# andrewmilson/ministark

Measured on NVIDIA H100. Metric: ntt_field_ops_per_s, higher is better.
Workload: dtype u64

## Files before the change

### ministark_b200/csrc/dft.cuh

```cuda
#pragma once
#include "field.cuh"

namespace msntt {
using namespace gl;

template <bool INV>
__host__ __device__ __forceinline__ constexpr u64 w16(int k) {
    constexpr u64 F[8] = {0x00000000FFFFFFFFULL, 0x0000000010000000ULL, 0xFEFFFFFF01000001ULL, 0xFFEFFFFF00000001ULL,
                          0xFFFFFFFEFFFF0001ULL, 0x00000FFFFFFFF000ULL, 0x0000010000000000ULL, 0x0000000000000010ULL};
    constexpr u64 I[8] = {0x00000000FFFFFFFFULL, 0xFFFFFFFEFFFFFFF1ULL, 0xFFFFFEFF00000001ULL, 0xFFFFEFFF00001001ULL,
                          0x0000000000010000ULL, 0x0010000000000000ULL, 0x00FFFFFFFF000000ULL, 0xFFFFFFFEF0000001ULL};
    return INV ? I[k] : F[k];
}

struct W16Shift {
    int m;
    bool neg;
};
template <bool INV>
__host__ __device__ constexpr W16Shift w16_shift(int k) {
    constexpr W16Shift F[8] = {{0, false}, {28, false}, {88, true}, {52, true}, {16, true}, {76, false}, {40, false}, {4, false}};
    constexpr W16Shift I[8] = {{0, false}, {4, true}, {40, true}, {76, true}, {16, false}, {52, false}, {88, false}, {28, true}};
    return INV ? I[k] : F[k];
}
__host__ __device__ constexpr u64 pow2_mod_p(int m) {
    return m < 64 ? (1ULL << m) : ((1ULL << (m - 32)) - (1ULL << (m - 64)));
}
template <bool INV, int K>
__host__ __device__ constexpr bool w16_shift_ok() {
    constexpr W16Shift s = w16_shift<INV>(K);
    constexpr u64 v = pow2_mod_p(s.m);
    return (s.neg ? P - v : v) == w16<INV>(K);
}
static_assert(w16_shift_ok<false, 1>() && w16_shift_ok<false, 2>() && w16_shift_ok<false, 3>() && w16_shift_ok<false, 4>() &&
              w16_shift_ok<false, 5>() && w16_shift_ok<false, 6>() && w16_shift_ok<false, 7>(), "forward 16th roots");
static_assert(w16_shift_ok<true, 1>() && w16_shift_ok<true, 2>() && w16_shift_ok<true, 3>() && w16_shift_ok<true, 4>() &&
              w16_shift_ok<true, 5>() && w16_shift_ok<true, 6>() && w16_shift_ok<true, 7>(), "inverse 16th roots");

template <int V>
struct IC {
    static constexpr int value = V;
    __host__ __device__ constexpr operator int() const { return V; }
};
template <int I, int N, typename F>
__device__ __forceinline__ void static_for(F &&f) {
    if constexpr (I < N) {
        f(IC<I>{});
        static_for<I + 1, N>(f);
    }
}
__host__ __device__ constexpr int brev_c(int k, int bits) {
    int r = 0;
    for (int b = 0; b < bits; b++) r |= ((k >> b) & 1) << (bits - 1 - b);
    return r;
}

template <int B, bool INV, int S, int A>
struct Bfly {
    static __device__ __forceinline__ void run(u64 (&x)[1 << B]) {
        constexpr int span = 1 << (B - S);
        if constexpr ((A & span) == 0) {
            constexpr int j = brev_c(A >> (B - S + 1), S - 1);
            const u64 u = x[A], v = x[A + span];
            if constexpr (j == 0) {
                if constexpr (S == 1) {
                    x[A] = add_lc(u, v);
                    x[A + span] = sub_lc(u, v);
                } else {
                    x[A] = add_ll(u, v);
                    x[A + span] = sub_ll(u, v);
                }
            } else {
#ifdef MS_DFT_CONST_MUL
                constexpr u64 w = w16<INV>(j * (16 >> S));
                const u64 t = mul(v, w);
                x[A] = add_lc(u, t);
                x[A + span] = sub_lc(u, t);
#else
                constexpr W16Shift sh = w16_shift<INV>(j * (16 >> S));
                const u64 t = mul_pow2<sh.m>(v);
                if constexpr (sh.neg) {
                    x[A] = sub_lc(u, t);
                    x[A + span] = add_lc(u, t);
                } else {
                    x[A] = add_lc(u, t);
                    x[A + span] = sub_lc(u, t);
                }
#endif
            }
        }
        if constexpr (A + 1 < (1 << B))
            Bfly<B, INV, S, A + 1>::run(x);
        else if constexpr (S < B)
            Bfly<B, INV, S + 1, 0>::run(x);
    }
};
template <int B, bool INV>
__device__ __forceinline__ void dft_regs(u64 (&x)[1 << B]) {
    Bfly<B, INV, 1, 0>::run(x);
}

}
```

### ministark_b200/csrc/field.cuh

```cuda
#pragma once
#ifndef __CUDACC_RTC__
#include <cstdint>
#endif

namespace gl {

typedef unsigned long long u64;
typedef unsigned int u32;

constexpr u64 P = 0xFFFFFFFF00000001ULL;
constexpr u64 EPS = 0xFFFFFFFFULL;
constexpr u64 ONE = EPS;
constexpr u64 R2 = 0xFFFFFFFE00000001ULL;
constexpr u64 TWO = 0x1FFFFFFFEULL;

#if defined(__CUDACC__)
#define GL_DEV __device__ __forceinline__
#define GL_HD __host__ __device__ __forceinline__
#else
#define GL_DEV inline
#define GL_HD inline
#endif

#if defined(__CUDACC__) && (defined(MS_CANON_MAD) || defined(MS_ADD_MAD))
static __constant__ u32 kEpsOperand = 0xFFFFFFFFu;
#endif
#if defined(__CUDA_ARCH__) && defined(MS_CANON_MAD)
__device__ __forceinline__ u64 canon(u64 x) {
    u64 r;
    asm("{\n\t.reg .u32 x0, x1, t0, t1, c;\n\tmov.b64 {x0, x1}, %1;\n\tadd.cc.u32 t0, x0, 0xffffffff;\n\taddc.cc.u32 t1, x1, 0;\n\t"
        "addc.u32 c, 0, 0;\n\tmad.wide.u32 %0, c, %2, %1;\n\t}"
        : "=l"(r) : "l"(x), "r"(kEpsOperand));
    return r;
}
#else
GL_HD u64 canon(u64 x) {
    u32 x0 = (u32)x, x1 = (u32)(x >> 32);
    const bool c = (x1 == 0xFFFFFFFFu) && (x0 != 0);
    x0 -= c ? 1u : 0u;
    x1 = c ? 0u : x1;
    return ((u64)x1 << 32) | x0;
}
#endif

GL_HD u64 add(u64 a, u64 b) {
    u64 s = a + b;
    u64 t = s + EPS;
    return (s < a || t < s) ? t : s;
}
GL_HD u64 sub(u64 a, u64 b) {
    u64 d = a - b;
    return a < b ? d - EPS : d;
}
GL_HD u64 neg(u64 a) { return a ? P - a : 0; }

#if defined(__CUDA_ARCH__)
__device__ __forceinline__ u64 pack64(u32 lo, u32 hi) { u64 r; asm("mov.b64 %0, {%1,%2};" : "=l"(r) : "r"(lo), "r"(hi)); return r; }
__device__ __forceinline__ void unpack64(u64 v, u32 &lo, u32 &hi) { asm("mov.b64 {%0,%1}, %2;" : "=r"(lo), "=r"(hi) : "l"(v)); }
#if defined(MS_ADD_MAD)
__device__ __forceinline__ u64 add_lc(u64 a, u64 t) {
    u32 a0, a1, t0, t1;
    u64 r;
    unpack64(a, a0, a1); unpack64(t, t0, t1);
    asm("{\n\t.reg .u32 s0, s1, c;\n\t.reg .u64 s;\n\tadd.cc.u32 s0, %1, %3;\n\taddc.cc.u32 s1, %2, %4;\n\taddc.u32 c, 0, 0;\n\t"
        "mov.b64 s, {s0, s1};\n\tmad.wide.u32 %0, c, %5, s;\n\t}"
        : "=l"(r) : "r"(a0), "r"(a1), "r"(t0), "r"(t1), "r"(kEpsOperand));
    return r;
}
#else
__device__ __forceinline__ u64 add_lc(u64 a, u64 t) {
    u32 a0, a1, t0, t1, s0, s1;
    unpack64(a, a0, a1); unpack64(t, t0, t1);
    asm("{\n\t.reg .u32 c;\n\tadd.cc.u32 %0, %2, %4;\n\taddc.cc.u32 %1, %3, %5;\n\taddc.u32 c, 0, 0;\n\t"
        "sub.cc.u32 %0, %0, c;\n\tsubc.u32 %1, %1, 0;\n\tadd.u32 %1, %1, c;\n\t}"
        : "=r"(s0), "=r"(s1) : "r"(a0), "r"(a1), "r"(t0), "r"(t1));
    return pack64(s0, s1);
}
#endif
__device__ __forceinline__ u64 sub_lc(u64 a, u64 t) {
    u32 a0, a1, t0, t1, s0, s1;
    unpack64(a, a0, a1); unpack64(t, t0, t1);
    asm("{\n\t.reg .u32 m;\n\tsub.cc.u32 %0, %2, %4;\n\tsubc.cc.u32 %1, %3, %5;\n\tsubc.u32 m, 0, 0;\n\t"
        "sub.cc.u32 %0, %0, m;\n\tsubc.u32 %1, %1, 0;\n\t}"
        : "=r"(s0), "=r"(s1) : "r"(a0), "r"(a1), "r"(t0), "r"(t1));
    return pack64(s0, s1);
}
__device__ __forceinline__ u64 add_ll(u64 a, u64 t) {
    u32 a0, a1, t0, t1, s0, s1;
    unpack64(a, a0, a1); unpack64(t, t0, t1);
    asm("{\n\t.reg .u32 c, m;\n\tadd.cc.u32 %0, %2, %4;\n\taddc.cc.u32 %1, %3, %5;\n\taddc.u32 c, 0, 0;\n\tsub.u32 m, 0, c;\n\t"
        "add.cc.u32 %0, %0, m;\n\taddc.cc.u32 %1, %1, 0;\n\taddc.u32 c, 0, 0;\n\tsub.u32 m, 0, c;\n\t"
        "add.cc.u32 %0, %0, m;\n\taddc.u32 %1, %1, 0;\n\t}"
        : "=r"(s0), "=r"(s1) : "r"(a0), "r"(a1), "r"(t0), "r"(t1));
    return pack64(s0, s1);
}
__device__ __forceinline__ u64 sub_ll(u64 a, u64 t) {
    u32 a0, a1, t0, t1, s0, s1;
    unpack64(a, a0, a1); unpack64(t, t0, t1);
    asm("{\n\t.reg .u32 m;\n\tsub.cc.u32 %0, %2, %4;\n\tsubc.cc.u32 %1, %3, %5;\n\tsubc.u32 m, 0, 0;\n\t"
        "sub.cc.u32 %0, %0, m;\n\tsubc.cc.u32 %1, %1, 0;\n\tsubc.u32 m, 0, 0;\n\t"
        "sub.cc.u32 %0, %0, m;\n\tsubc.u32 %1, %1, 0;\n\t}"
        : "=r"(s0), "=r"(s1) : "r"(a0), "r"(a1), "r"(t0), "r"(t1));
    return pack64(s0, s1);
}
#else
inline u64 add_lc(u64 a, u64 t) {
    u64 s = a + t;
    return s < a ? s + EPS : s;
}
inline u64 sub_lc(u64 a, u64 t) {
    u64 d = a - t;
    return a < t ? d - EPS : d;
}
inline u64 add_ll(u64 a, u64 b) {
    u64 s = a + b;
    if (s < a) { u64 s2 = s + EPS; s = s2 < s ? s2 + EPS : s2; }
    return s;
}
inline u64 sub_ll(u64 a, u64 b) {
    u64 d = a - b;
    if (a < b) { u64 d2 = d - EPS; d = d < EPS ? d2 - EPS : d2; }
    return d;
}
#endif

GL_HD u64 mont_reduce(u64 hi, u64 lo) {
#if defined(__CUDA_ARCH__)
    u32 r0, r1, r2, r3, q0, q1;
    unpack64(lo, r0, r1); unpack64(hi, r2, r3);
    asm("{\n\t.reg .u32 A1, e, B0, B1, m;\n\t"
        "add.cc.u32 A1, %3, %2;\n\taddc.u32 e, 0, 0;\n\tadd.u32 e, e, A1;\n\t"
        "sub.cc.u32 B0, %2, e;\n\tsubc.u32 B1, A1, 0;\n\t"
        "sub.cc.u32 %0, %4, B0;\n\tsubc.cc.u32 %1, %5, B1;\n\tsubc.u32 m, 0, 0;\n\t"
        "sub.cc.u32 %0, %0, m;\n\tsubc.u32 %1, %1, 0;\n\t}"
        : "=&r"(q0), "=&r"(q1) : "r"(r0), "r"(r1), "r"(r2), "r"(r3));
    return pack64(q0, q1);
#else
    u64 a = lo + (lo << 32);
    u64 e = a < lo;
    u64 b = a - (a >> 32) - e;
    u64 r = hi - b;
    return hi < b ? r - EPS : r;
#endif
}
GL_HD u64 mul(u64 a, u64 b) {
#if defined(__CUDA_ARCH__)
    return mont_reduce(__umul64hi(a, b), a * b);
#else
    unsigned __int128 x = (unsigned __int128)a * b;
    return mont_reduce((u64)(x >> 64), (u64)x);
#endif
}
template <int M>
GL_HD u64 mul_pow2(u64 x) {
    static_assert(M > 0 && M < 96, "shift out of range");
    if constexpr (M < 64) {
        return mont_reduce(x >> (64 - M), x << M);
    } else {
        constexpr int k = M - 64;
        const u64 lo = x << k, hi = x >> (64 - k);
        return canon(add_lc(lo, (hi << 32) - hi));
    }
}
GL_HD u64 sqr(u64 a) { return mul(a, a); }
GL_HD u64 to_mont(u64 x_canon) { return mul(x_canon, R2); }
GL_HD u64 from_mont(u64 w) { return mul(w, 1); }

GL_HD u64 pow(u64 a, u64 e) {
    u64 r = ONE;
    while (e) {
        if (e & 1) r = mul(r, a);
        a = sqr(a);
        e >>= 1;
    }
    return r;
}
GL_HD u64 inv(u64 a) {
    u64 x1 = a;
    u64 x2 = mul(sqr(x1), x1);
    u64 x3 = mul(sqr(x2), x1);
    u64 x6 = x3; for (int i = 0; i < 3; i++) x6 = sqr(x6); x6 = mul(x6, x3);
    u64 x12 = x6; for (int i = 0; i < 6; i++) x12 = sqr(x12); x12 = mul(x12, x6);
    u64 x24 = x12; for (int i = 0; i < 12; i++) x24 = sqr(x24); x24 = mul(x24, x12);
    u64 x30 = x24; for (int i = 0; i < 6; i++) x30 = sqr(x30); x30 = mul(x30, x6);
    u64 x31 = mul(sqr(x30), x1);
    u64 x32 = mul(sqr(x31), x1);
    u64 r = x31;
    for (int i = 0; i < 33; i++) r = sqr(r);
    return mul(r, x32);
}

struct Fq3 {
    u64 c0, c1, c2;
};
GL_HD Fq3 fq3(u64 a) { return Fq3{a, 0, 0}; }
GL_HD Fq3 add(Fq3 a, Fq3 b) { return Fq3{add(a.c0, b.c0), add(a.c1, b.c1), add(a.c2, b.c2)}; }
GL_HD Fq3 sub(Fq3 a, Fq3 b) { return Fq3{sub(a.c0, b.c0), sub(a.c1, b.c1), sub(a.c2, b.c2)}; }
GL_HD Fq3 neg(Fq3 a) { return Fq3{neg(a.c0), neg(a.c1), neg(a.c2)}; }
GL_HD Fq3 mul(Fq3 a, u64 b) { return Fq3{mul(a.c0, b), mul(a.c1, b), mul(a.c2, b)}; }
GL_HD Fq3 mul(Fq3 a, Fq3 b) {
    u64 v0 = mul(a.c0, b.c0), v1 = mul(a.c1, b.c1), v2 = mul(a.c2, b.c2);
    u64 x12 = sub(sub(mul(add(a.c1, a.c2), add(b.c1, b.c2)), v1), v2);
    u64 x01 = sub(sub(mul(add(a.c0, a.c1), add(b.c0, b.c1)), v0), v1);
    u64 x02 = sub(sub(mul(add(a.c0, a.c2), add(b.c0, b.c2)), v0), v2);
    return Fq3{add(v0, add(x12, x12)), add(x01, add(v2, v2)), add(x02, v1)};
}
GL_HD Fq3 sqr(Fq3 a) { return mul(a, a); }
GL_HD Fq3 pow(Fq3 a, u64 e) {
    Fq3 r = fq3(ONE);
    while (e) {
        if (e & 1) r = mul(r, a);
        a = sqr(a);
        e >>= 1;
    }
    return r;
}
GL_HD Fq3 inv(Fq3 a) {
    u64 s0 = sub(sqr(a.c0), mul(TWO, mul(a.c1, a.c2)));
    u64 s1 = sub(mul(TWO, sqr(a.c2)), mul(a.c0, a.c1));
    u64 s2 = sub(sqr(a.c1), mul(a.c0, a.c2));
    u64 nrm = add(mul(a.c0, s0), mul(TWO, add(mul(a.c2, s1), mul(a.c1, s2))));
    u64 ni = inv(nrm);
    return Fq3{mul(s0, ni), mul(s1, ni), mul(s2, ni)};
}

}
```

Measured before the change: 852.8 billion.

## Use lazy 96-bit limb arithmetic in register DFT to skip per-butterfly reduction

Replaces the per-butterfly modular repair in the radix-16 register DFT with unreduced 96-bit three-limb accumulation. A 2^7·p bias is added to the first element so subtractions stay non-negative, and reduction happens once at the end. Power-of-two twiddle multiplies become limb shifts with folding. This cuts ALU work per butterfly but raises register pressure (3 words per element), which could cause spills or lower occupancy.

```diff
diff --git a/ministark_b200/csrc/dft.cuh b/ministark_b200/csrc/dft.cuh
--- a/ministark_b200/csrc/dft.cuh
+++ b/ministark_b200/csrc/dft.cuh
@@ -95,9 +95,48 @@
             Bfly<B, INV, S + 1, 0>::run(x);
     }
 };
+#ifndef MS_DFT_REPAIR_EACH
+constexpr u64 kBiasLo = P << 7;
+constexpr u32 kBiasHi = (u32)(P >> 57);
+static_assert(kBiasHi == 127 && kBiasLo == 0xFFFFFF8000000080ULL, "2^7 p");
+template <int B, bool INV, int S, int A>
+struct BflyL {
+    static __host__ __device__ __forceinline__ void run(L96 (&x)[1 << B]) {
+        constexpr int span = 1 << (B - S);
+        if constexpr ((A & span) == 0) {
+            constexpr int j = brev_c(A >> (B - S + 1), S - 1);
+            const L96 u = x[A], v = x[A + span];
+            if constexpr (j == 0) {
+                x[A] = l96_add(u, v);
+                x[A + span] = l96_sub(u, v);
+            } else {
+                constexpr W16Shift sh = w16_shift<INV>(j * (16 >> S));
+                constexpr int K = sh.m >= 64 ? sh.m - 64 : sh.m + 32;
+                constexpr bool neg = sh.neg != (sh.m < 64);
+                const L96 t = l96_mul_pow2<K>(v);
+                x[A] = neg ? l96_sub(u, t) : l96_add(u, t);
+                x[A + span] = neg ? l96_add(u, t) : l96_sub(u, t);
+            }
+        }
+        if constexpr (A + 1 < (1 << B))
+            BflyL<B, INV, S, A + 1>::run(x);
+        else if constexpr (S < B)
+            BflyL<B, INV, S + 1, 0>::run(x);
+    }
+};
+#endif
+
 template <int B, bool INV>
-__device__ __forceinline__ void dft_regs(u64 (&x)[1 << B]) {
+__host__ __device__ __forceinline__ void dft_regs(u64 (&x)[1 << B]) {
+#ifdef MS_DFT_REPAIR_EACH
     Bfly<B, INV, 1, 0>::run(x);
+#else
+    L96 y[1 << B];
+    for (int i = 0; i < (1 << B); i++) y[i] = l96(x[i]);
+    y[0] = l96_add(y[0], L96{(u32)kBiasLo, (u32)(kBiasLo >> 32), kBiasHi});
+    BflyL<B, INV, 1, 0>::run(y);
+    for (int i = 0; i < (1 << B); i++) x[i] = l96_reduce(y[i]);
+#endif
 }
 
 }
diff --git a/ministark_b200/csrc/field.cuh b/ministark_b200/csrc/field.cuh
--- a/ministark_b200/csrc/field.cuh
+++ b/ministark_b200/csrc/field.cuh
@@ -123,6 +123,60 @@
     return d;
 }
 #endif
+
+struct L96 {
+    u32 w0, w1, w2;
+};
+GL_HD L96 l96(u64 x) { return L96{(u32)x, (u32)(x >> 32), 0u}; }
+#if defined(__CUDA_ARCH__)
+__device__ __forceinline__ L96 l96_add(L96 a, L96 b) {
+    L96 r;
+    asm("add.cc.u32 %0, %3, %6;\n\taddc.cc.u32 %1, %4, %7;\n\taddc.u32 %2, %5, %8;"
+        : "=r"(r.w0), "=r"(r.w1), "=r"(r.w2) : "r"(a.w0), "r"(a.w1), "r"(a.w2), "r"(b.w0), "r"(b.w1), "r"(b.w2));
+    return r;
+}
+__device__ __forceinline__ L96 l96_sub(L96 a, L96 b) {
+    L96 r;
+    asm("sub.cc.u32 %0, %3, %6;\n\tsubc.cc.u32 %1, %4, %7;\n\tsubc.u32 %2, %5, %8;"
+        : "=r"(r.w0), "=r"(r.w1), "=r"(r.w2) : "r"(a.w0), "r"(a.w1), "r"(a.w2), "r"(b.w0), "r"(b.w1), "r"(b.w2));
+    return r;
+}
+#else
+inline L96 l96_add(L96 a, L96 b) {
+    const u64 s0 = (u64)a.w0 + b.w0, s1 = (u64)a.w1 + b.w1 + (s0 >> 32);
+    return L96{(u32)s0, (u32)s1, a.w2 + b.w2 + (u32)(s1 >> 32)};
+}
+inline L96 l96_sub(L96 a, L96 b) {
+    const u64 d0 = (u64)a.w0 - b.w0, d1 = (u64)a.w1 - b.w1 - (d0 >> 63);
+    return L96{(u32)d0, (u32)d1, a.w2 - b.w2 - (u32)(d1 >> 63)};
+}
+#endif
+template <int K>
+GL_HD L96 l96_mul_pow2(L96 v) {
+    static_assert(K > 0 && K < 96, "shift out of range");
+    constexpr int q = K / 32, r = K % 32;
+    u32 y0, y1, y2, y3;
+    if constexpr (r == 0) {
+        y0 = v.w0, y1 = v.w1, y2 = v.w2, y3 = (u32)((int)v.w2 >> 31);
+    } else {
+        y0 = v.w0 << r;
+        y1 = (v.w1 << r) | (v.w0 >> (32 - r));
+        y2 = (v.w2 << r) | (v.w1 >> (32 - r));
+        y3 = (u32)((int)v.w2 >> (32 - r));
+    }
+    if constexpr (q == 0) {
+        const u32 s = (u32)((int)y3 >> 31);
+        return l96_sub(l96_sub(l96_add(L96{y0, y1, 0u}, L96{0u, y2, 0u}), L96{y2, 0u, 0u}), L96{y3, s, s});
+    } else if constexpr (q == 1) {
+        const u32 s = (u32)((int)y3 >> 31);
+        return l96_sub(l96_sub(L96{0u, y0, 0u}, L96{y1, 0u, 0u}), l96_sub(L96{y2, y3, s}, L96{0u, y1, 0u}));
+    } else {
+        return l96_sub(l96_sub(L96{0u, y0, 0u}, L96{y0, 0u, 0u}), L96{y1, y2, y3});
+    }
+}
+GL_HD u64 l96_reduce(L96 v) {
+    return add_lc(((u64)v.w1 << 32) | v.w0, (u64)v.w2 * 0xFFFFFFFFull);
+}
 
 GL_HD u64 mont_reduce(u64 hi, u64 lo) {
 #if defined(__CUDA_ARCH__)
diff --git a/profiles/ntt_sass_count.py b/profiles/ntt_sass_count.py
--- /dev/null
+++ b/profiles/ntt_sass_count.py
@@ -0,0 +1,89 @@
+#!/usr/bin/env python
+import collections
+import os
+import re
+import subprocess
+import sys
+import tempfile
+
+ROOT = os.path.dirname(os.path.dirname(os.path.abspath(__file__)))
+CSRC = os.path.join(ROOT, "ministark_b200", "csrc")
+NVCC = os.environ.get("NVCC", "/usr/local/cuda/bin/nvcc")
+ALU = ("IADD3", "LOP3", "SHF", "SEL", "ISETP", "LEA", "VIADD")
+PROBE = r"""
+#include "dft.cuh"
+using namespace msntt;
+template <bool INV> __global__ void probe_dft16(u64 *p) {
+    u64 x[16];
+    static_for<0, 16>([&](auto K) { x[K] = p[threadIdx.x + 256 * (int)K]; });
+    dft_regs<4, INV>(x);
+    static_for<0, 16>([&](auto K) { p[threadIdx.x + 256 * (int)K] = x[K]; });
+}
+template __global__ void probe_dft16<false>(u64 *);
+template __global__ void probe_dft16<true>(u64 *);
+"""
+
+
+def compile_cubin(src, extra, tmp):
+    out = os.path.join(tmp, os.path.basename(src) + ".cubin")
+    r = subprocess.run([NVCC, "-std=c++17", "-O3", "-gencode", "arch=compute_90a,code=sm_90a", "-cubin", "-I", CSRC,
+                        "-I", os.path.join(CSRC, "build"), "-Xptxas", "-v", *extra, "-o", out, src],
+                       capture_output=True, text=True, check=True)
+    spills, cur = {}, None
+    for line in r.stderr.splitlines():
+        m = re.search(r"Compiling entry function '(\w+)'", line) or re.search(r"Function properties for (\w+)", line)
+        if m:
+            cur = m.group(1)
+        m = re.search(r"(\d+) bytes spill stores", line)
+        if m and cur:
+            spills[cur] = int(m.group(1))
+        m = re.search(r"Used (\d+) registers", line)
+        if m and cur:
+            spills[cur] = (spills.get(cur, 0), int(m.group(1)))
+    return out, spills
+
+
+def sass_counts(cubin):
+    sass = subprocess.run(["cuobjdump", "-sass", cubin], capture_output=True, text=True, check=True).stdout
+    per, cur = collections.defaultdict(collections.Counter), None
+    for line in sass.splitlines():
+        m = re.match(r"\s*Function : (\w+)", line)
+        if m:
+            cur = m.group(1)
+            continue
+        m = re.match(r"\s*/\*[0-9a-f]{4,}\*/\s+(?:@!?U?P\w+\s+)?([A-Z0-9_.]+)", line)
+        if m and cur:
+            per[cur][m.group(1).split(".")[0]] += 1
+    return per
+
+
+def short_name(mangled):
+    m = re.search(r"(probe_dft16|ntt_tma_scatter_kernel|ntt_tma_kernel)I(.*?)EEv", mangled)
+    if not m:
+        return mangled
+    args = [a.replace("Li", "").replace("Lb", "") for a in re.findall(r"L[ib]\d+", m.group(2))]
+    return f"{m.group(1)}<{', '.join(args)}>"
+
+
+def main():
+    print("| build | kernel | ALU pipe | ALU / element | IMAD | all | registers | spill stores |")
+    print("|---|---|---|---|---|---|---|---|")
+    with tempfile.TemporaryDirectory() as tmp:
+        probe = os.path.join(tmp, "probe.cu")
+        with open(probe, "w") as f:
+            f.write(PROBE)
+        for label, extra in (("repair each butterfly (-DMS_DFT_REPAIR_EACH=1)", ["-DMS_DFT_REPAIR_EACH=1"]), ("96-bit limbs", [])):
+            for src in (probe, os.path.join(CSRC, "ntt_tma.cu")):
+                cubin, regs = compile_cubin(src, extra, tmp)
+                per = sass_counts(cubin)
+                for k in sorted(per):
+                    ops = per[k]
+                    alu = sum(v for op, v in ops.items() if op in ALU)
+                    imad = sum(v for op, v in ops.items() if op.startswith("IMAD"))
+                    sp, nr = regs.get(k, (0, None)) if isinstance(regs.get(k), tuple) else (regs.get(k, 0), None)
+                    name = short_name(k)
+                    print(f"| {label} | `{name}` | {alu} | {alu / 16:.1f} | {imad} | {sum(ops.values())} | {nr} | {sp} |")
+
+
+if __name__ == "__main__":
+    sys.exit(main())
```

Result: faster. 887.2 billion, median of 6 (+4.0%).
